# asarigun/mma

Measured on AMD Instinct MI355X. Metric: aggregated edges/sec (fwd+bwd) MultiMaskConv, higher is better.
Workload: dtype f32

## Files before the change

mma_amd/csrc/nc_fused.hip:

```cpp
#include "nc_shared.h"

#ifndef NC_FWD_UNROLL
#define NC_FWD_UNROLL(K) ((K) >= 3 ? 1 : 2)
#endif
#ifndef NC_BWD_UNROLL
#define NC_BWD_UNROLL(K) ((K) >= 3 ? 1 : 2)
#endif
#ifndef MMA_MIN_WAVES
#define MMA_MIN_WAVES 2
#endif
namespace mma {

template <class TT>
struct NcFwdParamsT {
  const float* x; int64_t ldx;
  const TT* P; int64_t ldp; const TT* Q; int64_t ldq;
  const int32_t* rowptr; const int32_t* col;
  const int4* items; int64_t n_items;
  float* partial; int64_t pstride;
  float* m; int64_t m_kstride;
  float* msum; int64_t ldms;
  float* T; uint8_t* sel; int64_t ldt;
  float* crow; int64_t ldc; uint32_t sel_slots;
  int H, HQ, K_total, k_base, lpr_log;
  uint32_t kinds, acts;
  DropParams drop;
  const int4* hubs; int64_t n_hubs; unsigned* sync; unsigned n_slots;
};
using NcFwdParams = NcFwdParamsT<float>;

__device__ __forceinline__ int kind_of(uint32_t kinds, int k) { return (kinds >> (4 * k)) & 0xF; }
__device__ __forceinline__ uint32_t sel_slot_of(uint32_t slots, int k) { return (slots >> (4 * k)) & 0xFu; }
template <int VEC>
__device__ __forceinline__ uint32_t crow_codes(const float* crow_row, uint32_t sel_slots, int k, int HQ, int c, uint32_t dflt) {
  const uint32_t sslot = sel_slot_of(sel_slots, k);
  return sslot != 0xFu ? ldb<VEC>(reinterpret_cast<const uint8_t*>(crow_row + 4 + (size_t)sslot * HQ) + c) : dflt;
}

__device__ __forceinline__ float nc_combine(int kind, float xi, float s, float deg, uint32_t& code) {
  code = 1;
  switch (kind) {
    case MMA_KIND_SUM: return xi + s;
    case MMA_KIND_MEAN: return (xi + s) / deg;
    case MMA_KIND_MAX: code = s > xi ? 1u : (s == xi ? 2u : 0u); return s > xi ? s : xi;
    case MMA_KIND_MIN: code = s < xi ? 1u : (s == xi ? 2u : 0u); return s < xi ? s : xi;
    default: {
      const float e = expf(kind == MMA_KIND_SOFTMAX ? s : -s);
      const float r = (e / e) * s;
      code = (r != r || (1.0f / e) > 3.402823466e38f) ? 3u : 1u;
      return r;
    }
  }
}

template <int VEC, bool SAVE, class PP>
__device__ __forceinline__ Vec<VEC> nc_fwd_write(const PP& p, int node, int k_abs, int c, const Vec<VEC>& xi,
                                                 const Vec<VEC>& s, const Vec<VEC>& t, float deg) {
  Vec<VEC> mo;
  uint32_t codes = 0;
  const int kind = kind_of(p.kinds, k_abs);
#pragma unroll
  for (int i = 0; i < VEC; ++i) {
    uint32_t code;
    mo.v[i] = nc_combine(kind, xi.v[i], s.v[i], deg, code);
    codes |= code << (8 * i);
  }
  if (p.m) stv<VEC>(p.m + (size_t)k_abs * p.m_kstride + (size_t)node * p.H + c, mo);
  if (SAVE) {
    const size_t o = (size_t)node * p.ldt + (size_t)k_abs * p.H + c;
    stv_nt<VEC>(p.T + o, t);
    if (p.sel) stb_nt<VEC>(p.sel + o, codes);
    if (p.crow && sel_slot_of(p.sel_slots, k_abs) != 0xFu) {
      uint32_t tf = 0;
#pragma unroll
      for (int i = 0; i < VEC; ++i) {
        const uint32_t code = (codes >> (8 * i)) & 0xFFu;
        tf |= (code == 1u ? 2u : (code == 2u ? 1u : (code == 3u ? 255u : 0u))) << (8 * i);
      }
      stb<VEC>(reinterpret_cast<uint8_t*>(p.crow + (size_t)node * p.ldc + 4 + (size_t)sel_slot_of(p.sel_slots, k_abs) * p.HQ) + c, tf);
    }
  }
  return mo;
}

template <int VEC, class PP>
__device__ __forceinline__ void nc_msum_store(const PP& p, int node, int c, Vec<VEC> ms, bool accumulate) {
  float* o = p.msum + (size_t)node * p.ldms + c;
  if (accumulate) {
    const Vec<VEC> prev = ldv<VEC>(o);
#pragma unroll
    for (int i = 0; i < VEC; ++i) ms.v[i] += prev.v[i];
  }
  if (accumulate) stv<VEC>(o, ms); else stv_nt<VEC>(o, ms);
}

template <int VEC, bool SAVE, class PP>
__device__ __forceinline__ void nc_fwd_finalize_body(const PP& p, const int4* hubs, int64_t n_hubs, const int64_t first, const int64_t step);

template <int K, int VEC, bool SAVE, int DM, bool MULTI, bool ONE = false, class TT>
__device__ __forceinline__ void nc_fwd_body(const NcFwdParamsT<TT>& p, const int bx, const int nbx) {
  const DropParams dp = (DM == MMA_DROP_HASH || DM == MMA_DROP_HASH16) ? drop_resolve(p.drop) : p.drop;
  uint32_t mult[K], mult2[K];
#pragma unroll
  for (int k = 0; k < K; ++k) { mult[k] = drop_mask_mult(p.k_base + k); mult2[k] = drop_mask_mult2(p.k_base + k); }
  constexpr int U = NC_FWD_UNROLL(K);
  const int lane = threadIdx.x & (kWave - 1);
  const int lpr = 1 << p.lpr_log;
  const int G = MULTI ? lpr : kWave;
  const int epg = G >> p.lpr_log;
  const int gpw = kWave / G;
  const int grp = MULTI ? lane / G : 0;
  const int gl = lane & (G - 1);
  const int gbase = grp * G;
  const int sub = gl >> p.lpr_log;
  const int c = ((int)blockIdx.y * lpr + (lane & (lpr - 1))) * VEC;
  const bool fvalid = c < p.H;
  const int cc = fvalid ? c : 0;
  const int waves_per_block = kBlock / kWave;
  const int64_t stride = (int64_t)nbx * waves_per_block;
  const int64_t n_witems = (p.n_items + gpw - 1) / gpw;

  for (int64_t it0 = (int64_t)bx * waves_per_block + (threadIdx.x >> 6); it0 < n_witems; it0 += stride) {
    int node, ebeg, eend, slot;
    bool ivalid = true;
    if (MULTI) {
      const int64_t idx = it0 * gpw + grp;
      ivalid = idx < p.n_items;
      const int4 item = p.items[ivalid ? idx : 0];
      node = item.x; ebeg = item.y; eend = ivalid ? item.z : item.y; slot = item.w;
    } else {
      const int4 item = p.items[__builtin_amdgcn_readfirstlane((int)it0)];
      node = __builtin_amdgcn_readfirstlane(item.x);
      ebeg = __builtin_amdgcn_readfirstlane(item.y);
      eend = __builtin_amdgcn_readfirstlane(item.z);
      slot = __builtin_amdgcn_readfirstlane(item.w);
    }
    const int len = eend - ebeg;
    int maxlen = len;
    if (MULTI) {
      for (int off = G; off < kWave; off <<= 1) maxlen = max(maxlen, __shfl_xor(maxlen, off, kWave));
      maxlen = __builtin_amdgcn_readfirstlane(maxlen);
    }

    const Vec<VEC> xi = ldv<VEC>(p.x + row_off(node, p.ldx) + cc);
    Vec<VEC> pk[K], acc[K], tac[K];
#pragma unroll
    for (int k = 0; k < K; ++k) {
      pk[k] = ldt_nt<VEC>(p.P + row_off(node, p.ldp) + (size_t)(p.k_base + k) * p.H + cc);
      acc[k] = vzero<VEC>();
      tac[k] = vzero<VEC>();
    }

    for (int base = 0; base < maxlen; base += G) {
      const int cnt = min(G, max(len - base, 0));
      const int ucnt = min(G, maxlen - base);
      const int myj = (gl < cnt) ? p.col[ebeg + base + gl] : 0;
      for (int t0 = 0; t0 < ucnt; t0 += U * epg) {
        int tt[U]; bool ev[U]; Vec<VEC> xj[U]; Vec<VEC> qv[U][K];
#pragma unroll
        for (int u = 0; u < U; ++u) {
          tt[u] = t0 + u * epg + sub;
          ev[u] = tt[u] < cnt;
          const int j = __shfl(myj, gbase + (tt[u] & (G - 1)), kWave);
          const int jj = ev[u] ? j : node;
          xj[u] = ldv<VEC>(p.x + row_off(jj, p.ldx) + cc);
          const TT* qrow = p.Q + row_off(jj, p.ldq) + cc;
#pragma unroll
          for (int k = 0; k < K; ++k)
            qv[u][k] = ldt<VEC>(qrow + (size_t)(p.k_base + k) * p.H);
        }
#pragma unroll
        for (int u = 0; u < U; ++u) {
#pragma unroll
          for (int i = 0; i < VEC; ++i) xj[u].v[i] = ev[u] ? xj[u].v[i] : 0.f;
          const uint32_t eu = (uint32_t)(ev[u] ? ebeg + base + tt[u] : 0);
          const uint32_t hw = (DM == MMA_DROP_HASH || DM == MMA_DROP_HASH16) ? drop_base_word(dp, eu, cc >> 2) : 0u;
#pragma unroll
          for (int k = 0; k < K; ++k) {
            const bool raw = (p.acts >> (p.k_base + k)) & 1u;
            float f[VEC];
            if (DM == MMA_DROP_HASH) {
              drop_unpack<VEC>(dp, drop_mask_word(hw, k == 0 ? p.k_base : 1, mult[k]), cc, f);
            } else if (DM == MMA_DROP_HASH16) {
              drop_unpack16<VEC>(dp, drop_mask_word(hw, k == 0 ? p.k_base : 1, mult[k]), drop_low_word(hw, mult2[k]), cc, f);
            } else if (DM == MMA_DROP_EXPLICIT) {
              drop_explicit<VEC>(dp, eu, p.k_base + k, cc, p.H, f);
            } else {
#pragma unroll
              for (int i = 0; i < VEC; ++i) f[i] = 1.f;
            }
#pragma unroll
            for (int i = 0; i < VEC; ++i) {
              const float z = pk[k].v[i] + qv[u][k].v[i];
              float a, da;
              if (raw) { a = z; da = 1.f; }
              else { a = sigmoid_fast(z); da = a - a * a; }
              const float w = f[i] * xj[u].v[i];
              acc[k].v[i] = fmaf(a, w, acc[k].v[i]);
              if (SAVE) tac[k].v[i] = fmaf(da, w, tac[k].v[i]);
            }
          }
        }
      }
    }

    for (int off = G / 2; off >= lpr; off >>= 1) {
#pragma unroll
      for (int k = 0; k < K; ++k)
#pragma unroll
        for (int i = 0; i < VEC; ++i) {
          acc[k].v[i] += __shfl_xor(acc[k].v[i], off, kWave);
          if (SAVE) tac[k].v[i] += __shfl_xor(tac[k].v[i], off, kWave);
        }
    }

    if (sub == 0 && fvalid && ivalid) {
      if (slot < 0) {
        const float deg = (float)max(p.rowptr[node + 1] - p.rowptr[node], 1);
        Vec<VEC> ms = vzero<VEC>();
#pragma unroll
        for (int k = 0; k < K; ++k) {
          const Vec<VEC> mo = nc_fwd_write<VEC, SAVE>(p, node, p.k_base + k, c, xi, acc[k], tac[k], deg);
#pragma unroll
          for (int i = 0; i < VEC; ++i) ms.v[i] += mo.v[i];
        }
        if (p.msum) nc_msum_store<VEC>(p, node, c, ms, p.k_base > 0);
        if (SAVE && p.crow && c == 0 && p.k_base == 0) p.crow[(size_t)node * p.ldc] = 1.f / deg;
      } else {
        float* ps = p.partial + (size_t)slot * p.pstride;
#pragma unroll
        for (int k = 0; k < K; ++k) {
          stv<VEC>(ps + (size_t)(p.k_base + k) * p.H + c, acc[k]);
          if (SAVE) stv<VEC>(ps + (size_t)(p.K_total + p.k_base + k) * p.H + c, tac[k]);
        }
      }
    }
    if (ONE) {
      const bool wrote = ivalid && slot >= 0;
      if (__builtin_amdgcn_ballot_w64(wrote) != 0) {
        __builtin_amdgcn_fence(__ATOMIC_RELEASE, "agent");
        unsigned ticket = 0u;
        if (wrote && gl == 0) ticket = atomicAdd(p.sync, 1u) + 1u;
        if (__builtin_amdgcn_ballot_w64(ticket == p.n_slots) != 0) {
          __builtin_amdgcn_fence(__ATOMIC_ACQUIRE, "agent");
          nc_fwd_finalize_body<VEC, SAVE>(p, p.hubs, p.n_hubs, lane, kWave);
          if (lane == 0) *p.sync = 0u;
        }
      }
    }
  }
}

template <int K, int VEC, bool SAVE, int DM, bool MULTI, class TT = float>
__global__ __launch_bounds__(kBlock, (K <= 4 ? MMA_MIN_WAVES : 1)) void nc_fwd_kernel(const NcFwdParamsT<TT> p) {
  nc_fwd_body<K, VEC, SAVE, DM, MULTI>(p, (int)blockIdx.x, (int)gridDim.x);
}

template <int VEC, bool SAVE, class PP>
__device__ __forceinline__ void nc_fwd_finalize_body(const PP& p, const int4* hubs, int64_t n_hubs, const int64_t first, const int64_t step) {
  const int per_row = (p.H + VEC - 1) / VEC;
  const int64_t total = n_hubs * per_row;
  for (int64_t idx = first; idx < total; idx += step) {
    const int c = (int)(idx % per_row) * VEC;
    const int4 hub = hubs[idx / per_row];
    const int node = hub.x;
    const Vec<VEC> xi = ldv<VEC>(p.x + (size_t)node * p.ldx + c);
    const float deg = (float)max(p.rowptr[node + 1] - p.rowptr[node], 1);
    Vec<VEC> ms = vzero<VEC>();
    for (int k = 0; k < p.K_total; ++k) {
      Vec<VEC> s = vzero<VEC>(), t = vzero<VEC>();
      constexpr int kAhead = 8;
      for (int sl0 = hub.y; sl0 < hub.z; sl0 += kAhead) {
        Vec<VEC> a[kAhead], b[kAhead];
#pragma unroll
        for (int u = 0; u < kAhead; ++u) {
          const float* ps = p.partial + (size_t)min(sl0 + u, hub.z - 1) * p.pstride;
          a[u] = ldv<VEC>(ps + (size_t)k * p.H + c);
          if (SAVE) b[u] = ldv<VEC>(ps + (size_t)(p.K_total + k) * p.H + c);
        }
#pragma unroll
        for (int u = 0; u < kAhead; ++u) {
          if (sl0 + u < hub.z) {
#pragma unroll
            for (int i = 0; i < VEC; ++i) s.v[i] += a[u].v[i];
            if (SAVE) {
#pragma unroll
              for (int i = 0; i < VEC; ++i) t.v[i] += b[u].v[i];
            }
          }
        }
      }
      const Vec<VEC> mo = nc_fwd_write<VEC, SAVE>(p, node, k, c, xi, s, t, deg);
#pragma unroll
      for (int i = 0; i < VEC; ++i) ms.v[i] += mo.v[i];
    }
    if (p.msum) nc_msum_store<VEC>(p, node, c, ms, false);
    if (SAVE && p.crow && c == 0) p.crow[(size_t)node * p.ldc] = 1.f / deg;
  }
}
template <int VEC, bool SAVE, class TT = float>
__global__ __launch_bounds__(kBlock) void nc_fwd_finalize_kernel(const NcFwdParamsT<TT> p, const int4* hubs, int64_t n_hubs) {
  nc_fwd_finalize_body<VEC, SAVE>(p, hubs, n_hubs, (int64_t)blockIdx.x * blockDim.x + threadIdx.x, (int64_t)gridDim.x * blockDim.x);
}

struct NcSmallPlan { int64_t n_wave_items; int blocks_a; };

template <int K, int VEC, bool SAVE, int DM, class TT = float>
__global__ __launch_bounds__(kBlock, (K <= 4 ? MMA_MIN_WAVES : 1)) void nc_fwd_small_kernel(const NcFwdParamsT<TT> p, const NcSmallPlan sp) {
  if ((int)blockIdx.x < sp.blocks_a) {
    NcFwdParamsT<TT> q = p;
    q.n_items = sp.n_wave_items;
    nc_fwd_body<K, VEC, SAVE, DM, false, true>(q, (int)blockIdx.x, sp.blocks_a);
  } else {
    NcFwdParamsT<TT> q = p;
    q.items = p.items + sp.n_wave_items; q.n_items = p.n_items - sp.n_wave_items;
    nc_fwd_body<K, VEC, SAVE, DM, true, true>(q, (int)blockIdx.x - sp.blocks_a, (int)gridDim.x - sp.blocks_a);
  }
}

struct NcBwdNodeParams {
  const float* g; int64_t g_kstride, ldgr;
  const uint8_t* sel; const float* T; int64_t ldt; const int32_t* rowptr;
  float* gs; int64_t ldgs; float* gP; int64_t ldgp; float* gxs; int64_t ldgx;
  int64_t N; int H, K; uint32_t kinds;
  const float* crow; int64_t ldc; int HQ; uint32_t sel_slots;
  uint32_t* rowmax;
};

__device__ __forceinline__ void combine_grad_tf(int kind, uint32_t tf, float inv_deg, float& fs, float& fx) {
  switch (kind) {
    case MMA_KIND_SUM: fs = 1.f; fx = 1.f; break;
    case MMA_KIND_MEAN: fs = inv_deg; fx = inv_deg; break;
    case MMA_KIND_MAX:
    case MMA_KIND_MIN: fs = 0.5f * (float)tf; fx = 1.f - fs; break;
    default: fs = tf == 255u ? __builtin_nanf("") : 1.f; fx = 0.f; break;
  }
}

template <int VEC>
__global__ __launch_bounds__(kBlock) void nc_bwd_node_kernel(const NcBwdNodeParams p) {
  const int per_row = (p.H + VEC - 1) / VEC;
  const int64_t total = p.N * per_row;
  for (int64_t idx = (int64_t)blockIdx.x * blockDim.x + threadIdx.x; idx < total; idx += (int64_t)gridDim.x * blockDim.x) {
    const int64_t node = idx / per_row;
    const int c = (int)(idx % per_row) * VEC;
    const float deg = (float)max(p.rowptr[node + 1] - p.rowptr[node], 1);
    const float inv_deg = 1.f / deg;
    Vec<VEC> gk[MMA_MAX_K], tk[MMA_MAX_K];
    uint32_t ck[MMA_MAX_K];
    const bool shared_g = p.g_kstride == 0;
#pragma unroll
    for (int k = 0; k < MMA_MAX_K; ++k) {
      if (k < p.K) {
        const size_t o = (size_t)node * p.ldt + (size_t)k * p.H + c;
        if (k == 0 || !shared_g) gk[k] = ldv_nt<VEC>(p.g + (size_t)k * p.g_kstride + (size_t)node * p.ldgr + c);
        tk[k] = ldv_nt<VEC>(p.T + o);
        if (p.crow) {
          ck[k] = crow_codes<VEC>(p.crow + (size_t)node * p.ldc, p.sel_slots, k, p.HQ, c, 0u);
        } else {
          ck[k] = ldb_nt<VEC>(p.sel + o);
        }
      }
    }
    Vec<VEC> gx = vzero<VEC>();
    float mxp = 0.f;
#pragma unroll
    for (int k = 0; k < MMA_MAX_K; ++k) {
      if (k < p.K) {
        const int kind = kind_of(p.kinds, k);
        const Vec<VEC> g = shared_g ? gk[0] : gk[k];
        const Vec<VEC> t = tk[k];
        const uint32_t codes = ck[k];
        Vec<VEC> gsv, gpv;
#pragma unroll
        for (int i = 0; i < VEC; ++i) {
          uint32_t tf = (codes >> (8 * i)) & 0xFFu;
          if (!p.crow) tf = tf == 1u ? 2u : (tf == 2u ? 1u : (tf == 3u ? 255u : 0u));
          float fs, fx;
          combine_grad_tf(kind, tf, inv_deg, fs, fx);
          gsv.v[i] = g.v[i] * fs;
          gpv.v[i] = gsv.v[i] * t.v[i];
          gx.v[i] = fmaf(g.v[i], fx, gx.v[i]);
          mxp = fmaxf(mxp, fabsf(gpv.v[i]));
        }
        if (p.gs) stv<VEC>(p.gs + (size_t)node * p.ldgs + (size_t)k * p.H + c, gsv);
        stv_nt<VEC>(p.gP + (size_t)node * p.ldgp + (size_t)k * p.H + c, gpv);
      }
    }
    stv_nt<VEC>(p.gxs + (size_t)node * p.ldgx + c, gx);
    if (p.rowmax) {
      if ((per_row & (per_row - 1)) == 0 && per_row <= kWave) {
        for (int off = per_row >> 1; off > 0; off >>= 1) mxp = fmaxf(mxp, __shfl_xor(mxp, off, kWave));
        if ((idx & (per_row - 1)) == 0 && mxp > 0.f) atomicMax(p.rowmax + node, __float_as_uint(mxp));
      } else if (mxp > 0.f) {
        atomicMax(p.rowmax + node, __float_as_uint(mxp));
      }
    }
  }
}

template <class TT>
struct NcBwdParamsT {
  const float* x; int64_t ldx;
  const TT* P; int64_t ldp; const TT* Q; int64_t ldq;
  const float* gs; int64_t ldg; const float* gxs; int64_t ldgx;
  const float* g; int64_t ldgg; const float* crow; int64_t ldc; uint32_t sel_slots; uint32_t kinds;
  const float* T; int64_t ldt; float* gP; int64_t ldgp; int64_t n_targets;
  const int32_t* t_col; const int32_t* t_eid;
  const int4* items; int64_t n_items;
  float* partial; int64_t pstride;
  float* gQ; int64_t ldgq; float* gx; int64_t ldgxo;
  int H, HQ, K_total, k_base, lpr_log;
  uint32_t acts;
  DropParams drop;
  int first_pass;
  uint32_t* rowmax;
  const int4* hubs; int64_t n_hubs; unsigned* sync; unsigned n_slots;
};
using NcBwdParams = NcBwdParamsT<float>;

template <int VEC, class PP>
__device__ __forceinline__ Vec<VEC> nc_bwd_epilogue(const PP& p, int node, int c, int k0, int nk, float& mx) {
  const Vec<VEC> g = ldv_nt<VEC>(p.g + row_off(node, p.ldgg) + c);
  const float* crow = p.crow + row_off(node, p.ldc);
  const float inv_deg = crow[0];
  Vec<VEC> gxd = vzero<VEC>();
  Vec<VEC> tk[MMA_MAX_K]; uint32_t ck[MMA_MAX_K];
#pragma unroll
  for (int k = 0; k < MMA_MAX_K; ++k) {
    if (k < nk) {
      tk[k] = ldv_nt<VEC>(p.T + row_off(node, p.ldt) + (size_t)(k0 + k) * p.H + c);
      ck[k] = crow_codes<VEC>(crow, p.sel_slots, k0 + k, p.HQ, c, 0u);
    }
  }
#pragma unroll
  for (int k = 0; k < MMA_MAX_K; ++k) {
    if (k < nk) {
      const int kind = kind_of(p.kinds, k0 + k);
      Vec<VEC> gpv;
#pragma unroll
      for (int i = 0; i < VEC; ++i) {
        float fs, fx;
        combine_grad_tf(kind, (ck[k] >> (8 * i)) & 0xFFu, inv_deg, fs, fx);
        gpv.v[i] = (g.v[i] * fs) * tk[k].v[i];
        gxd.v[i] = fmaf(g.v[i], fx, gxd.v[i]);
        mx = fmaxf(mx, fabsf(gpv.v[i]));
      }
      stv_nt<VEC>(p.gP + row_off(node, p.ldgp) + (size_t)(k0 + k) * p.H + c, gpv);
    }
  }
  return gxd;
}

template <int VEC, class PP>
__device__ __forceinline__ void nc_bwd_finalize_body(const PP& p, const int4* hubs, int64_t n_hubs, const int64_t first, const int64_t step);

template <int K, int VEC, int DM, bool SHARED, bool MULTI, bool EPI, bool ONE = false, class TT>
__device__ __forceinline__ void nc_bwd_body(const NcBwdParamsT<TT>& p, const int bx, const int nbx) {
  constexpr bool DROP = DM != MMA_DROP_NONE;
  const DropParams dp = (DM == MMA_DROP_HASH || DM == MMA_DROP_HASH16) ? drop_resolve(p.drop) : p.drop;
  uint32_t mult[K], mult2[K];
#pragma unroll
  for (int k = 0; k < K; ++k) { mult[k] = drop_mask_mult(p.k_base + k); mult2[k] = drop_mask_mult2(p.k_base + k); }
  constexpr int U = NC_BWD_UNROLL(K);
  const int lane = threadIdx.x & (kWave - 1);
  const int lpr = 1 << p.lpr_log;
  const int G = MULTI ? lpr : kWave;
  const int epg = G >> p.lpr_log;
  const int gpw = kWave / G;
  const int grp = MULTI ? lane / G : 0;
  const int gl = lane & (G - 1);
  const int gbase = grp * G;
  const int sub = gl >> p.lpr_log;
  const int c = ((int)blockIdx.y * lpr + (lane & (lpr - 1))) * VEC;
  const bool fvalid = c < p.H;
  const int cc = fvalid ? c : 0;
  const int waves_per_block = kBlock / kWave;
  const int64_t stride = (int64_t)nbx * waves_per_block;
  const int64_t n_witems = (p.n_items + gpw - 1) / gpw;

  for (int64_t it0 = (int64_t)bx * waves_per_block + (threadIdx.x >> 6); it0 < n_witems; it0 += stride) {
    int node, ebeg, eend, slot;
    bool ivalid = true;
    if (MULTI) {
      const int64_t idx = it0 * gpw + grp;
      ivalid = idx < p.n_items;
      const int4 item = p.items[ivalid ? idx : 0];
      node = item.x; ebeg = item.y; eend = ivalid ? item.z : item.y; slot = item.w;
    } else {
      const int4 item = p.items[__builtin_amdgcn_readfirstlane((int)it0)];
      node = __builtin_amdgcn_readfirstlane(item.x);
      ebeg = __builtin_amdgcn_readfirstlane(item.y);
      eend = __builtin_amdgcn_readfirstlane(item.z);
      slot = __builtin_amdgcn_readfirstlane(item.w);
    }
    const int len = eend - ebeg;
    int maxlen = len;
    if (MULTI) {
      for (int off = G; off < kWave; off <<= 1) maxlen = max(maxlen, __shfl_xor(maxlen, off, kWave));
      maxlen = __builtin_amdgcn_readfirstlane(maxlen);
    }

    const Vec<VEC> xj = ldv_nt<VEC>(p.x + row_off(node, p.ldx) + cc);
    Vec<VEC> qk[K], aq[K];
    Vec<VEC> ax = vzero<VEC>();
#pragma unroll
    for (int k = 0; k < K; ++k) {
      qk[k] = ldt_nt<VEC>(p.Q + row_off(node, p.ldq) + (size_t)(p.k_base + k) * p.H + cc);
      aq[k] = vzero<VEC>();
    }

    for (int base = 0; base < maxlen; base += G) {
      const int cnt = min(G, max(len - base, 0));
      const int ucnt = min(G, maxlen - base);
      const int myi = (gl < cnt) ? p.t_col[ebeg + base + gl] : ((gl == 0 && len > 0) ? p.t_col[ebeg] : 0);
      const int mye = (DROP && gl < cnt) ? p.t_eid[ebeg + base + gl] : 0;
      for (int t0 = 0; t0 < ucnt; t0 += U * epg) {
        int tt[U]; bool ev[U]; uint32_t eid[U]; Vec<VEC> gv[U][SHARED ? 1 : K]; Vec<VEC> pv[U][K];
        uint32_t codes[U][K]; float idg[U];
#pragma unroll
        for (int u = 0; u < U; ++u) {
          tt[u] = t0 + u * epg + sub;
          ev[u] = tt[u] < cnt;
          const int tl = min(tt[u], max(cnt - 1, 0));
          const int ii = __shfl(myi, gbase + (tl & (G - 1)), kWave);
          eid[u] = DROP ? (uint32_t)__shfl(mye, gbase + (tl & (G - 1)), kWave) : 0u;
          if (SHARED) {
            gv[u][0] = ldv<VEC>(p.g + row_off(ii, p.ldgg) + cc);
            const float* crow = p.crow + row_off(ii, p.ldc);
            idg[u] = crow[0];
#pragma unroll
            for (int k = 0; k < K; ++k) {
              codes[u][k] = crow_codes<VEC>(crow, p.sel_slots, p.k_base + k, p.HQ, cc, 0x02020202u);
            }
          }
          const TT* prow = p.P + row_off(ii, p.ldp) + cc;
          const float* grow = SHARED ? nullptr : p.gs + row_off(ii, p.ldg) + cc;
#pragma unroll
          for (int k = 0; k < K; ++k) {
            const size_t o = (size_t)(p.k_base + k) * p.H;
            if (!SHARED) gv[u][k] = ldv<VEC>(grow + o);
            pv[u][k] = ldt<VEC>(prow + o);
          }
        }
#pragma unroll
        for (int u = 0; u < U; ++u) {
          const bool live = ev[u];
#pragma unroll
          for (int kk = 0; kk < (SHARED ? 1 : K); ++kk)
#pragma unroll
            for (int i = 0; i < VEC; ++i) gv[u][kk].v[i] = live ? gv[u][kk].v[i] : 0.f;
          const uint32_t hw = (DM == MMA_DROP_HASH || DM == MMA_DROP_HASH16) ? drop_base_word(dp, eid[u], cc >> 2) : 0u;
#pragma unroll
          for (int k = 0; k < K; ++k) {
            const bool raw = (p.acts >> (p.k_base + k)) & 1u;
            const int kind = SHARED ? kind_of(p.kinds, p.k_base + k) : 0;
            const float kscale = 0.5f * (kind == MMA_KIND_MEAN ? idg[u] : 1.f);
            float f[VEC];
            if (DM == MMA_DROP_HASH) {
              drop_unpack<VEC>(dp, drop_mask_word(hw, k == 0 ? p.k_base : 1, mult[k]), cc, f);
            } else if (DM == MMA_DROP_HASH16) {
              drop_unpack16<VEC>(dp, drop_mask_word(hw, k == 0 ? p.k_base : 1, mult[k]), drop_low_word(hw, mult2[k]), cc, f);
            } else if (DM == MMA_DROP_EXPLICIT) {
              drop_explicit<VEC>(dp, eid[u], p.k_base + k, cc, p.H, f);
            } else {
#pragma unroll
              for (int i = 0; i < VEC; ++i) f[i] = 1.f;
            }
#pragma unroll
            for (int i = 0; i < VEC; ++i) {
              const float z = pv[u][k].v[i] + qk[k].v[i];
              float a, da;
              if (raw) { a = z; da = 1.f; }
              else { a = sigmoid_fast(z); da = a - a * a; }
              float gsv;
              if (SHARED) {
                const uint32_t tf = (codes[u][k] >> (8 * i)) & 0xFFu;
                float cf = (float)tf;
                if (kind >= MMA_KIND_SOFTMAX && tf == 255u) cf = __builtin_nanf("");
                gsv = gv[u][0].v[i] * (cf * kscale);
              } else {
                gsv = gv[u][k].v[i];
              }
              const float w = f[i] * gsv;
              aq[k].v[i] = fmaf(da, w, aq[k].v[i]);
              ax.v[i] = fmaf(a, w, ax.v[i]);
            }
          }
        }
      }
    }

    const bool writer = sub == 0 && fvalid && ivalid;
    const bool tgt = EPI && writer && slot < 0 && (int64_t)node < p.n_targets;
    Vec<VEC> gxd = vzero<VEC>();
    float mxp = 0.f;
    if (EPI) { if (tgt) gxd = nc_bwd_epilogue<VEC>(p, node, c, p.k_base, K, mxp); }

    for (int off = G / 2; off >= lpr; off >>= 1) {
#pragma unroll
      for (int i = 0; i < VEC; ++i) {
        ax.v[i] += __shfl_xor(ax.v[i], off, kWave);
#pragma unroll
        for (int k = 0; k < K; ++k) aq[k].v[i] += __shfl_xor(aq[k].v[i], off, kWave);
      }
    }
    if (len == 0) {
      ax = vzero<VEC>();
#pragma unroll
      for (int k = 0; k < K; ++k) aq[k] = vzero<VEC>();
    }

    if (p.rowmax) {
      float mxq = mxp;
      if (writer && slot < 0) {
#pragma unroll
        for (int k = 0; k < K; ++k)
#pragma unroll
          for (int i = 0; i < VEC; ++i) mxq = fmaxf(mxq, fabsf(xj.v[i] * aq[k].v[i]));
      }
      for (int off = lpr >> 1; off > 0; off >>= 1) mxq = fmaxf(mxq, __shfl_xor(mxq, off, kWave));
      if (sub == 0 && (lane & (lpr - 1)) == 0 && ivalid && slot < 0 && mxq > 0.f) atomicMax(p.rowmax + node, __float_as_uint(mxq));
    }
    if (writer) {
      if (slot < 0) {
#pragma unroll
        for (int k = 0; k < K; ++k) {
          Vec<VEC> o;
#pragma unroll
          for (int i = 0; i < VEC; ++i) o.v[i] = xj.v[i] * aq[k].v[i];
          stv_nt<VEC>(p.gQ + row_off(node, p.ldgq) + (size_t)(p.k_base + k) * p.H + c, o);
        }
        Vec<VEC> g0;
        if (EPI) {
          g0 = gxd;
          if (!p.first_pass) {
            const Vec<VEC> prev = ldv<VEC>(p.gx + row_off(node, p.ldgxo) + c);
#pragma unroll
            for (int i = 0; i < VEC; ++i) g0.v[i] += prev.v[i];
          }
        } else {
          g0 = p.first_pass ? ldv_nt<VEC>(p.gxs + row_off(node, p.ldgx) + c) : ldv<VEC>(p.gx + row_off(node, p.ldgxo) + c);
        }
        Vec<VEC> o;
#pragma unroll
        for (int i = 0; i < VEC; ++i) o.v[i] = g0.v[i] + ax.v[i];
        stv_nt<VEC>(p.gx + row_off(node, p.ldgxo) + c, o);
      } else {
        float* ps = p.partial + (size_t)slot * p.pstride;
#pragma unroll
        for (int k = 0; k < K; ++k) stv<VEC>(ps + (size_t)(p.k_base + k) * p.H + c, aq[k]);
        float* px = ps + (size_t)p.K_total * p.H + c;
        if (p.first_pass) stv<VEC>(px, ax);
        else {
          const Vec<VEC> prev = ldv<VEC>(px);
          Vec<VEC> o;
#pragma unroll
          for (int i = 0; i < VEC; ++i) o.v[i] = prev.v[i] + ax.v[i];
          stv<VEC>(px, o);
        }
      }
    }
    if (ONE) {
      const bool wrote = ivalid && slot >= 0;
      if (__builtin_amdgcn_ballot_w64(wrote) != 0) {
        __builtin_amdgcn_fence(__ATOMIC_RELEASE, "agent");
        unsigned ticket = 0u;
        if (wrote && gl == 0) ticket = atomicAdd(p.sync, 1u) + 1u;
        if (__builtin_amdgcn_ballot_w64(ticket == p.n_slots) != 0) {
          __builtin_amdgcn_fence(__ATOMIC_ACQUIRE, "agent");
          nc_bwd_finalize_body<VEC>(p, p.hubs, p.n_hubs, lane, kWave);
          if (lane == 0) *p.sync = 0u;
        }
      }
    }
  }
}

template <int K, int VEC, int DM, bool SHARED, bool MULTI, bool EPI, class TT = float>
__global__ __launch_bounds__(kBlock, (K <= 4 ? MMA_MIN_WAVES : 1)) void nc_bwd_kernel(const NcBwdParamsT<TT> p) {
  nc_bwd_body<K, VEC, DM, SHARED, MULTI, EPI>(p, (int)blockIdx.x, (int)gridDim.x);
}

template <int VEC, class PP>
__device__ __forceinline__ void nc_bwd_finalize_body(const PP& p, const int4* hubs, int64_t n_hubs, const int64_t first, const int64_t step) {
  const int per_row = (p.H + VEC - 1) / VEC;
  const bool epi = p.T != nullptr;
  const int64_t total = n_hubs * (p.K_total + 1) * per_row;
  for (int64_t idx = first; idx < total; idx += step) {
    const int c = (int)(idx % per_row) * VEC;
    const int k = (int)((idx / per_row) % (p.K_total + 1));
    const int4 hub = hubs[idx / ((int64_t)per_row * (p.K_total + 1))];
    Vec<VEC> s = vzero<VEC>();
    constexpr int kAhead = 8;
    for (int sl0 = hub.y; sl0 < hub.z; sl0 += kAhead) {
      Vec<VEC> a[kAhead];
#pragma unroll
      for (int u = 0; u < kAhead; ++u) a[u] = ldv<VEC>(p.partial + (size_t)min(sl0 + u, hub.z - 1) * p.pstride + (size_t)k * p.H + c);
#pragma unroll
      for (int u = 0; u < kAhead; ++u) {
        if (sl0 + u < hub.z) {
#pragma unroll
          for (int i = 0; i < VEC; ++i) s.v[i] += a[u].v[i];
        }
      }
    }
    const int node = hub.x;
    const bool tgt = epi && (int64_t)node < p.n_targets;
    Vec<VEC> o;
    if (k < p.K_total) {
      const Vec<VEC> xj = ldv<VEC>(p.x + (size_t)node * p.ldx + c);
      float mxq = 0.f;
      if (tgt) nc_bwd_epilogue<VEC>(p, node, c, k, 1, mxq);
#pragma unroll
      for (int i = 0; i < VEC; ++i) o.v[i] = xj.v[i] * s.v[i];
      stv_nt<VEC>(p.gQ + (size_t)node * p.ldgq + (size_t)k * p.H + c, o);
      if (p.rowmax) {
#pragma unroll
        for (int i = 0; i < VEC; ++i) mxq = fmaxf(mxq, fabsf(o.v[i]));
        if (mxq > 0.f) atomicMax(p.rowmax + node, __float_as_uint(mxq));
      }
    } else {
      Vec<VEC> g0 = vzero<VEC>();
      if (tgt) {
        const Vec<VEC> g = ldv<VEC>(p.g + row_off(node, p.ldgg) + c);
        const float* crow = p.crow + row_off(node, p.ldc);
        const float inv_deg = crow[0];
        for (int kk = 0; kk < p.K_total; ++kk) {
          const uint32_t sslot = sel_slot_of(p.sel_slots, kk);
          const uint32_t ck = sslot != 0xFu ? ldb<VEC>(reinterpret_cast<const uint8_t*>(crow + 4 + (size_t)sslot * p.HQ) + c) : 0u;
#pragma unroll
          for (int i = 0; i < VEC; ++i) {
            float fs, fx;
            combine_grad_tf(kind_of(p.kinds, kk), (ck >> (8 * i)) & 0xFFu, inv_deg, fs, fx);
            g0.v[i] = fmaf(g.v[i], fx, g0.v[i]);
          }
        }
      } else if (!epi) {
        g0 = ldv<VEC>(p.gxs + (size_t)node * p.ldgx + c);
      }
#pragma unroll
      for (int i = 0; i < VEC; ++i) o.v[i] = g0.v[i] + s.v[i];
      stv<VEC>(p.gx + (size_t)node * p.ldgxo + c, o);
    }
  }
}
template <int VEC, class TT = float>
__global__ __launch_bounds__(kBlock) void nc_bwd_finalize_kernel(const NcBwdParamsT<TT> p, const int4* hubs, int64_t n_hubs) {
  nc_bwd_finalize_body<VEC>(p, hubs, n_hubs, (int64_t)blockIdx.x * blockDim.x + threadIdx.x, (int64_t)gridDim.x * blockDim.x);
}

template <int K, int VEC, int DM, bool EPI, class TT = float>
__global__ __launch_bounds__(kBlock, (K <= 4 ? MMA_MIN_WAVES : 1)) void nc_bwd_small_kernel(const NcBwdParamsT<TT> p, const NcSmallPlan sp) {
  if ((int)blockIdx.x < sp.blocks_a) {
    NcBwdParamsT<TT> q = p;
    q.n_items = sp.n_wave_items;
    nc_bwd_body<K, VEC, DM, true, false, EPI, true>(q, (int)blockIdx.x, sp.blocks_a);
  } else {
    NcBwdParamsT<TT> q = p;
    q.items = p.items + sp.n_wave_items; q.n_items = p.n_items - sp.n_wave_items;
    nc_bwd_body<K, VEC, DM, true, true, EPI, true>(q, (int)blockIdx.x - sp.blocks_a, (int)gridDim.x - sp.blocks_a);
  }
}

static int pack_codes(const uint8_t* kind_host, const uint8_t* act_host, int K, uint32_t* kinds, uint32_t* acts) {
  *kinds = 0; *acts = 0;
  for (int k = 0; k < K; ++k) {
    if (kind_host) {
      if (kind_host[k] > MMA_KIND_SOFTMIN) return fail(1, "kind[%d]=%d is not an MMA_KIND_* code", k, (int)kind_host[k]);
      *kinds |= (uint32_t)kind_host[k] << (4 * k);
    }
    if (act_host) {
      if (act_host[k] > MMA_ACT_RAW) return fail(1, "act[%d]=%d is not an MMA_ACT_* code", k, (int)act_host[k]);
      *acts |= (uint32_t)act_host[k] << k;
    }
  }
  return 0;
}

static int64_t fill_sel_slots(const uint8_t* kind_host, int K, int H, uint32_t* slots) {
  int n = 0;
  *slots = 0xFFFFFFFFu;
  for (int k = 0; k < K; ++k)
    if (kind_host[k] >= MMA_KIND_MAX) { *slots = (*slots & ~(0xFu << (4 * k))) | ((uint32_t)n << (4 * k)); ++n; }
  return ((4 + (int64_t)n * (((int64_t)H + 3) / 4)) + 3) & ~(int64_t)3;
}

template <class F> static void with_k(int Ks, F&& f) {
  switch (Ks) {
    case 1: f(ic<1>{}); break;
    case 2: f(ic<2>{}); break;
    case 3: f(ic<3>{}); break;
    case 4: f(ic<4>{}); break;
    default: f(ic<8>{}); break;
  }
}
template <class F> static void with_form(int vec, int part, F&& f) {
  with_flag(vec == 4, [&](auto v4) { with_flag(part != 0, [&](auto multi) { f(ic<decltype(v4)::value ? 4 : 1>{}, multi); }); });
}

template <int VEC, bool MULTI, class TT>
static void launch_fwd(int Ks, const NcFwdParamsT<TT>& p, dim3 grid, bool save, int dm, hipStream_t st) {
  with_k(Ks, [&](auto k) { with_flag(save, [&](auto sv) { with_dm(dm, [&](auto d) {
    hipLaunchKernelGGL((nc_fwd_kernel<decltype(k)::value, VEC, decltype(sv)::value, decltype(d)::value, MULTI, TT>), grid, dim3(kBlock), 0, st, p);
  }); }); });
}
template <int VEC, bool MULTI, class TT>
static void launch_bwd(int Ks, const NcBwdParamsT<TT>& p, dim3 grid, int dm, hipStream_t st) {
  with_k(Ks, [&](auto k) { with_dm(dm, [&](auto d) { with_flag(p.gs == nullptr, [&](auto shared) { with_flag(p.T != nullptr, [&](auto epi) {
    constexpr bool SHARED = decltype(shared)::value, EPI = SHARED && decltype(epi)::value;
    hipLaunchKernelGGL((nc_bwd_kernel<decltype(k)::value, VEC, decltype(d)::value, SHARED, MULTI, EPI, TT>), grid, dim3(kBlock), 0, st, p);
  }); }); }); });
}

template <class TT>
static void launch_fwd_small(int K, const NcFwdParamsT<TT>& p, const NcSmallPlan& sp, dim3 grid, bool save, int dm, hipStream_t st) {
  with_k(K, [&](auto k) { with_flag(save, [&](auto sv) { with_dm<false>(dm, [&](auto d) {
    hipLaunchKernelGGL((nc_fwd_small_kernel<decltype(k)::value, 4, decltype(sv)::value, decltype(d)::value, TT>), grid, dim3(kBlock), 0, st, p, sp);
  }); }); });
}
template <class TT>
static void launch_bwd_small(int K, const NcBwdParamsT<TT>& p, const NcSmallPlan& sp, dim3 grid, int dm, hipStream_t st) {
  with_k(K, [&](auto k) { with_flag(p.T != nullptr, [&](auto epi) { with_dm<false>(dm, [&](auto d) {
    hipLaunchKernelGGL((nc_bwd_small_kernel<decltype(k)::value, 4, decltype(d)::value, decltype(epi)::value, TT>), grid, dim3(kBlock), 0, st, p, sp);
  }); }); });
}
static bool small_plan(int32_t* sync, int K, const Geometry& g, int dm, int64_t n_items, int64_t n_wave_items, int64_t n_hubs, int64_t n_slots,
                       int64_t finalize_elems, NcSmallPlan* sp, dim3* grid) {
  const bool one_slice = K <= 4 || K == 8;
  if (!sync || !one_slice || g.vec != 4 || g.chunks != 1 || dm == MMA_DROP_EXPLICIT || finalize_elems > 4096 || n_slots >= (1LL << 31)) return false;
  const int64_t n_group = n_items - n_wave_items;
  if (n_hubs == 0 && (n_wave_items == 0 || n_group == 0)) return false;
  const int ipw = kWave >> g.lpr_log;
  const unsigned ba = n_wave_items > 0 ? item_grid(n_wave_items, 1, 1).x : 0u;
  const unsigned bb = n_group > 0 ? item_grid(n_group, 1, ipw).x : 0u;
  *sp = NcSmallPlan{n_wave_items, (int)ba};
  *grid = dim3(ba + bb, 1, 1);
  return true;
}

static int next_slice(int remaining) { return remaining >= 8 ? 8 : (remaining >= 4 ? 4 : remaining); }

static int nc_common_checks(int64_t N, int64_t E, int32_t H, int32_t K) {
  if (int rc = nc_range_checks(N, E)) return rc;
  MMA_REQUIRE(H >= 1 && K >= 1 && K <= MMA_MAX_K, "H=%d K=%d unsupported (1<=K<=%d)", H, K, MMA_MAX_K);
  return 0;
}
template <class Params>
static void nc_set_hubs(Params& p, const int32_t* hubs, int64_t n_hubs, int32_t* sync, int64_t n_slots) {
  p.hubs = reinterpret_cast<const int4*>(hubs); p.n_hubs = n_hubs; p.sync = reinterpret_cast<unsigned*>(sync); p.n_slots = (unsigned)n_slots;
}
template <class Params, class F>
static void nc_for_slices(Params& p, int64_t n_wave_items, int K, const Geometry& g, F&& f) {
  const int4* all_items = p.items;
  const int64_t n_items = p.n_items;
  for (int part = 0; part < 2; ++part) {
    const int64_t cnt = part == 0 ? n_wave_items : n_items - n_wave_items;
    if (cnt <= 0) continue;
    p.items = all_items + (part == 0 ? 0 : n_wave_items);
    p.n_items = cnt;
    const dim3 grid = item_grid(cnt, g.chunks, part == 0 ? 1 : (kWave >> g.lpr_log));
    for (int k0 = 0; k0 < K;) {
      const int ks = next_slice(K - k0);
      p.k_base = k0;
      f(part, k0, ks, grid);
      k0 += ks;
    }
  }
}

}

using namespace mma;

template <class TT>
static int nc_fused_fwd(
    const float* x, int64_t ldx, const TT* P, int64_t ldp, const TT* Q, int64_t ldq,
    const int32_t* rowptr, const int32_t* col,
    const int32_t* items, int64_t n_items, int64_t n_wave_items, const int32_t* hubs, int64_t n_hubs,
    float* partial, int64_t n_slots, float* m, float* m_sum, int64_t ldms, float* T, uint8_t* sel, int64_t ldt,
    float* crow, int64_t ldc,
    int64_t N, int64_t E, int32_t H, int32_t K, const uint8_t* kind_host, const uint8_t* act_host,
    int32_t drop_mode, uint32_t drop_thr, uint64_t seed, const uint64_t* seed_dev, int64_t drop_edge_base, const uint8_t* keep,
    int32_t* sync, void* stream) {
  if (int rc = nc_common_checks(N, E, H, K)) return rc;
  MMA_REQUIRE(ldx >= H && ldp >= (int64_t)K * H && ldq >= (int64_t)K * H, "row pitch too small: ldx=%lld ldp=%lld ldq=%lld",
              (long long)ldx, (long long)ldp, (long long)ldq);
  MMA_REQUIRE(T != nullptr || (sel == nullptr && crow == nullptr), "sel / crow are saved next to T: give T too");
  MMA_REQUIRE(T == nullptr || sel != nullptr || crow != nullptr, "T needs the selection state beside it: sel (N,K*H), crow (N,ldc), or both");
  MMA_REQUIRE(T == nullptr || ldt >= (int64_t)K * H, "ldt=%lld too small", (long long)ldt);
  MMA_REQUIRE(ldx < (1LL << 31) && ldp < (1LL << 31) && ldq < (1LL << 31) && ldt < (1LL << 31) && ldc < (1LL << 31), "row pitch out of range");
  if (int rc = nc_item_checks(n_items, n_wave_items, hubs, n_hubs, partial, n_slots)) return rc;
  if (N == 0 || n_items == 0) return 0;
  MMA_REQUIRE(x && P && Q && rowptr && items && kind_host && act_host, "NULL argument");
  MMA_REQUIRE(m != nullptr || m_sum != nullptr, "give m (K,N,H), m_sum (N,H), or both");
  MMA_REQUIRE(m_sum == nullptr || ldms >= H, "ldms=%lld too small", (long long)ldms);
  MMA_REQUIRE(E == 0 || col != nullptr, "NULL col");
  if (int rc = nc_item_alignment(items, hubs)) return rc;
  uint32_t kinds, acts;
  if (int rc = pack_codes(kind_host, act_host, K, &kinds, &acts)) return rc;
// ... 232 lines not shown
```

Baseline: 754.7 million.

## Prefetch next work item and its first column indices in MULTI gather loops

In the multi-group forward and backward gather kernels, the next item descriptor and its first batch of column/edge indices are now loaded one iteration ahead. These loads are issued before the shuffle reduction and epilogue so their latency overlaps with work on the current item, with asm barriers placed where the values must have arrived. The forward path also hoists the rowptr loads used for the degree. The backward epilogue is split into a load phase, which issues its loads unconditionally using a dummy address for non-target lanes, followed by a full waitcnt and a compute/store phase. The cost is extra register pressure, and some redundant loads are issued for non-target lanes.

New measurement: 761.1 million (median of 6 runs). Within noise of the previous version (+0.9%).

```diff
diff --git a/mma_amd/csrc/nc_fused.hip b/mma_amd/csrc/nc_fused.hip
--- a/mma_amd/csrc/nc_fused.hip
+++ b/mma_amd/csrc/nc_fused.hip
@@ -29,6 +29,11 @@
 };
 using NcFwdParams = NcFwdParamsT<float>;
 
+__device__ __forceinline__ void nc_landed(int& a) { asm volatile("" : "+v"(a)); }
+__device__ __forceinline__ void nc_landed(int& a, int& b) { asm volatile("" : "+v"(a), "+v"(b)); }
+__device__ __forceinline__ void nc_landed(int& a, int& b, int& c) { asm volatile("" : "+v"(a), "+v"(b), "+v"(c)); }
+__device__ __forceinline__ void nc_all_landed() { __builtin_amdgcn_s_waitcnt(0x0F70); }
+
 __device__ __forceinline__ int kind_of(uint32_t kinds, int k) { return (kinds >> (4 * k)) & 0xF; }
 __device__ __forceinline__ uint32_t sel_slot_of(uint32_t slots, int k) { return (slots >> (4 * k)) & 0xFu; }
 template <int VEC>
@@ -120,14 +125,28 @@
   const int64_t stride = (int64_t)nbx * waves_per_block;
   const int64_t n_witems = (p.n_items + gpw - 1) / gpw;
 
+  int4 nitem = make_int4(0, 0, 0, 0);
+  int nj = 0;
+  int64_t gidx = ((int64_t)bx * waves_per_block + (threadIdx.x >> 6)) * gpw + grp;
+  const int64_t gstep = stride * gpw;
+  if (MULTI) {
+    if (gidx - grp < p.n_items) {
+      nitem = p.items[gidx < p.n_items ? gidx : 0];
+      if (gidx < p.n_items && gl < min(G, nitem.z - nitem.y)) nj = p.col[nitem.y + gl];
+    }
+    nc_landed(nj);
+  }
+
   for (int64_t it0 = (int64_t)bx * waves_per_block + (threadIdx.x >> 6); it0 < n_witems; it0 += stride) {
     int node, ebeg, eend, slot;
     bool ivalid = true;
+    int myj0 = 0;
     if (MULTI) {
-      const int64_t idx = it0 * gpw + grp;
-      ivalid = idx < p.n_items;
-      const int4 item = p.items[ivalid ? idx : 0];
-      node = item.x; ebeg = item.y; eend = ivalid ? item.z : item.y; slot = item.w;
+      ivalid = gidx < p.n_items;
+      node = nitem.x; ebeg = nitem.y; eend = ivalid ? nitem.z : nitem.y; slot = nitem.w;
+      myj0 = nj;
+      gidx += gstep;
+      nitem = p.items[gidx < p.n_items ? gidx : 0];
     } else {
       const int4 item = p.items[__builtin_amdgcn_readfirstlane((int)it0)];
       node = __builtin_amdgcn_readfirstlane(item.x);
@@ -154,7 +173,8 @@
     for (int base = 0; base < maxlen; base += G) {
       const int cnt = min(G, max(len - base, 0));
       const int ucnt = min(G, maxlen - base);
-      const int myj = (gl < cnt) ? p.col[ebeg + base + gl] : 0;
+      if (MULTI) __builtin_assume(ucnt > 0);
+      const int myj = (MULTI && base == 0) ? myj0 : ((gl < cnt) ? p.col[ebeg + base + gl] : 0);
       for (int t0 = 0; t0 < ucnt; t0 += U * epg) {
         int tt[U]; bool ev[U]; Vec<VEC> xj[U]; Vec<VEC> qv[U][K];
 #pragma unroll
@@ -204,6 +224,13 @@
       }
     }
 
+    int rp0 = 0, rp1 = 1;
+    if (MULTI) {
+      rp0 = p.rowptr[node]; rp1 = p.rowptr[node + 1];
+      nj = 0;
+      if (gidx < p.n_items && gl < min(G, nitem.z - nitem.y)) nj = p.col[nitem.y + gl];
+    }
+
     for (int off = G / 2; off >= lpr; off >>= 1) {
 #pragma unroll
       for (int k = 0; k < K; ++k)
@@ -214,9 +241,10 @@
         }
     }
 
+    if (MULTI) nc_landed(nj, rp0, rp1);
     if (sub == 0 && fvalid && ivalid) {
       if (slot < 0) {
-        const float deg = (float)max(p.rowptr[node + 1] - p.rowptr[node], 1);
+        const float deg = (float)max(MULTI ? rp1 - rp0 : p.rowptr[node + 1] - p.rowptr[node], 1);
         Vec<VEC> ms = vzero<VEC>();
 #pragma unroll
         for (int k = 0; k < K; ++k) {
@@ -452,6 +480,46 @@
   return gxd;
 }
 
+template <int VEC>
+struct NcBwdEpiRows { Vec<VEC> g; float inv_deg; Vec<VEC> tk[MMA_MAX_K]; uint32_t ck[MMA_MAX_K]; };
+
+template <int VEC, class PP>
+__device__ __forceinline__ void nc_bwd_epilogue_load(const PP& p, int node, int c, int k0, int nk, NcBwdEpiRows<VEC>& r, const float* alt) {
+  r.g = ldv_nt<VEC>(alt ? alt : p.g + row_off(node, p.ldgg) + c);
+  const float* crow = p.crow + row_off(node, p.ldc);
+  r.inv_deg = *(alt ? alt : crow);
+#pragma unroll
+  for (int k = 0; k < MMA_MAX_K; ++k) {
+    if (k < nk) {
+      r.tk[k] = ldv_nt<VEC>(alt ? alt : p.T + row_off(node, p.ldt) + (size_t)(k0 + k) * p.H + c);
+      const uint32_t sslot = sel_slot_of(p.sel_slots, k0 + k);
+      const uint8_t* cp = alt ? reinterpret_cast<const uint8_t*>(alt) : reinterpret_cast<const uint8_t*>(crow + 4 + (size_t)sslot * p.HQ) + c;
+      r.ck[k] = sslot != 0xFu ? ldb<VEC>(cp) : 0u;
+    }
+  }
+}
+template <int VEC, class PP>
+__device__ __forceinline__ Vec<VEC> nc_bwd_epilogue_store(const PP& p, int node, int c, int k0, int nk, float& mx, const NcBwdEpiRows<VEC>& r) {
+  Vec<VEC> gxd = vzero<VEC>();
+#pragma unroll
+  for (int k = 0; k < MMA_MAX_K; ++k) {
+    if (k < nk) {
+      const int kind = kind_of(p.kinds, k0 + k);
+      Vec<VEC> gpv;
+#pragma unroll
+      for (int i = 0; i < VEC; ++i) {
+        float fs, fx;
+        combine_grad_tf(kind, (r.ck[k] >> (8 * i)) & 0xFFu, r.inv_deg, fs, fx);
+        gpv.v[i] = (r.g.v[i] * fs) * r.tk[k].v[i];
+        gxd.v[i] = fmaf(r.g.v[i], fx, gxd.v[i]);
+        mx = fmaxf(mx, fabsf(gpv.v[i]));
+      }
+      stv_nt<VEC>(p.gP + row_off(node, p.ldgp) + (size_t)(k0 + k) * p.H + c, gpv);
+    }
+  }
+  return gxd;
+}
+
 template <int VEC, class PP>
 __device__ __forceinline__ void nc_bwd_finalize_body(const PP& p, const int4* hubs, int64_t n_hubs, const int64_t first, const int64_t step);
 
@@ -479,14 +547,31 @@
   const int64_t stride = (int64_t)nbx * waves_per_block;
   const int64_t n_witems = (p.n_items + gpw - 1) / gpw;
 
+  int4 nitem = make_int4(0, 0, 0, 0);
+  int ni = 0, ne = 0;
+  int64_t gidx = ((int64_t)bx * waves_per_block + (threadIdx.x >> 6)) * gpw + grp;
+  const int64_t gstep = stride * gpw;
+  if (MULTI) {
+    if (gidx - grp < p.n_items) {
+      nitem = p.items[gidx < p.n_items ? gidx : 0];
+      if (gidx < p.n_items && gl < min(G, nitem.z - nitem.y)) {
+        ni = p.t_col[nitem.y + gl];
+        if (DROP) ne = p.t_eid[nitem.y + gl];
+      }
+    }
+    nc_landed(ni, ne);
+  }
+
   for (int64_t it0 = (int64_t)bx * waves_per_block + (threadIdx.x >> 6); it0 < n_witems; it0 += stride) {
     int node, ebeg, eend, slot;
     bool ivalid = true;
+    int myi0 = 0, mye0 = 0;
     if (MULTI) {
-      const int64_t idx = it0 * gpw + grp;
-      ivalid = idx < p.n_items;
-      const int4 item = p.items[ivalid ? idx : 0];
-      node = item.x; ebeg = item.y; eend = ivalid ? item.z : item.y; slot = item.w;
+      ivalid = gidx < p.n_items;
+      node = nitem.x; ebeg = nitem.y; eend = ivalid ? nitem.z : nitem.y; slot = nitem.w;
+      myi0 = ni; mye0 = ne;
+      gidx += gstep;
+      nitem = p.items[gidx < p.n_items ? gidx : 0];
     } else {
       const int4 item = p.items[__builtin_amdgcn_readfirstlane((int)it0)];
       node = __builtin_amdgcn_readfirstlane(item.x);
@@ -513,8 +598,9 @@
     for (int base = 0; base < maxlen; base += G) {
       const int cnt = min(G, max(len - base, 0));
       const int ucnt = min(G, maxlen - base);
-      const int myi = (gl < cnt) ? p.t_col[ebeg + base + gl] : ((gl == 0 && len > 0) ? p.t_col[ebeg] : 0);
-      const int mye = (DROP && gl < cnt) ? p.t_eid[ebeg + base + gl] : 0;
+      if (MULTI) __builtin_assume(ucnt > 0);
+      const int myi = (MULTI && base == 0) ? myi0 : ((gl < cnt) ? p.t_col[ebeg + base + gl] : ((gl == 0 && len > 0) ? p.t_col[ebeg] : 0));
+      const int mye = (MULTI && base == 0) ? mye0 : ((DROP && gl < cnt) ? p.t_eid[ebeg + base + gl] : 0);
       for (int t0 = 0; t0 < ucnt; t0 += U * epg) {
         int tt[U]; bool ev[U]; uint32_t eid[U]; Vec<VEC> gv[U][SHARED ? 1 : K]; Vec<VEC> pv[U][K];
         uint32_t codes[U][K]; float idg[U];
@@ -591,11 +677,27 @@
       }
     }
 
+    if (MULTI) {
+      ni = 0; ne = 0;
+      if (gidx < p.n_items && gl < min(G, nitem.z - nitem.y)) {
+        ni = p.t_col[nitem.y + gl];
+        if (DROP) ne = p.t_eid[nitem.y + gl];
+      }
+    }
+
     const bool writer = sub == 0 && fvalid && ivalid;
     const bool tgt = EPI && writer && slot < 0 && (int64_t)node < p.n_targets;
     Vec<VEC> gxd = vzero<VEC>();
     float mxp = 0.f;
-    if (EPI) { if (tgt) gxd = nc_bwd_epilogue<VEC>(p, node, c, p.k_base, K, mxp); }
+    if (EPI && MULTI) {
+      NcBwdEpiRows<VEC> er;
+      nc_bwd_epilogue_load<VEC>(p, node, cc, p.k_base, K, er, tgt ? nullptr : p.x + row_off(node, p.ldx) + cc);
+      nc_all_landed();
+      if (tgt) gxd = nc_bwd_epilogue_store<VEC>(p, node, c, p.k_base, K, mxp, er);
+    } else {
+      if (MULTI) nc_landed(ni, ne);
+      if (EPI) { if (tgt) gxd = nc_bwd_epilogue<VEC>(p, node, c, p.k_base, K, mxp); }
+    }
 
     for (int off = G / 2; off >= lpr; off >>= 1) {
 #pragma unroll
```
